# 2InfinityN6eyond/AbsoluteTrack

Hardware: AMD Instinct MI355X
Metric: hand-frames/sec (higher is better)
Workload: dtype f32 (backbone products as two fp16 pieces per operand, fp32 accumulation); 1 GPU; 4 fisheye cameras x 2 hands per frame, 2 views per hand, 96x96 crops, known-skeleton path, full hot path (resample+backbone+head+FK) + all-gather of records; frames_per_gpu=1024, src_image=480x636 u8 x 4 cameras, parallelism=frame-shard x1, world=1, backend=none (single process), outputs_finite=True

## Files before the change

### absolutetrack_amd/_native.py

```python
import contextlib
import ctypes
import os
from typing import Dict, Optional, Tuple

import numpy as np
import torch

from . import arch

_HERE = os.path.dirname(os.path.abspath(__file__))
LIB_PATH = os.path.join(_HERE, "libumetrack_hip.so")

EXPORTS = (
    "ut_weight_blob_floats", "ut_create", "ut_destroy", "ut_last_error", "ut_reserve",
    "ut_set_backbone_chunk", "ut_warp_crops", "ut_backbone", "ut_fuse_temporal_regress",
    "ut_reset_memory", "ut_get_memory", "ut_fk", "ut_gen_crop_cameras", "ut_gen_crop_matrices",
    "ut_resample_homography", "ut_keypoint_metrics", "ut_profile_begin", "ut_profile_end", "ut_profile_end_by_kind",
    "ut_set_index_checks", "ut_poll_status", "ut_warp_backbone", "ut_set_latency_mode", "ut_set_conv_arithmetic",
    "ut_set_backbone_lanes", "ut_status_snapshot", "ut_warp_map", "ut_set_block_fusion", "ut_set_resident_weights",
    "ut_canonical_backbone_weights", "ut_set_split_scale", "ut_calibrate_split", "ut_get_split_calibration",
    "ut_gen_crop_cameras_from_window_points", "ut_get_split_adaptations",
    "ut_mesh_create", "ut_mesh_destroy", "ut_mesh_counts", "ut_skin_mesh",
)

UT_MODE_KNOWN, UT_MODE_UNKNOWN = 0, 1
UT_REMAP_CV2_FIXED, UT_REMAP_FLOAT = 0, 1
UT_CHECK_SYNC, UT_CHECK_DEFERRED = 0, 1
SPLIT_SCALE_MODES = {"calibrated": 0, "dynamic": 1, "adaptive": 2}

_lib = None


class NativeLibraryError(RuntimeError):
    pass


def load_library() -> ctypes.CDLL:
    global _lib
    if _lib is not None:
        return _lib
    if not os.path.exists(LIB_PATH):
        raise NativeLibraryError(
            f"{LIB_PATH} not found: build it with `python -c 'import __graft_entry__ as g; g.build()'` "
            "(hipcc --offload-arch=gfx950).  There is no CPU fallback for the hot path.")
    lib = ctypes.CDLL(LIB_PATH)
    vp, i32, f32p = ctypes.c_void_p, ctypes.c_int, ctypes.c_void_p
    lib.ut_weight_blob_floats.restype = ctypes.c_size_t
    lib.ut_weight_blob_floats.argtypes = []
    lib.ut_create.restype = i32
    lib.ut_create.argtypes = [i32, vp, ctypes.c_size_t, ctypes.POINTER(vp)]
    lib.ut_destroy.restype = i32
    lib.ut_destroy.argtypes = [vp]
# ... 23 lines not shown
    lib.ut_mesh_destroy.restype = i32
    lib.ut_mesh_destroy.argtypes = [vp]
    lib.ut_mesh_counts.restype = i32
    lib.ut_mesh_counts.argtypes = [vp, ctypes.POINTER(i32), ctypes.POINTER(i32)]
    lib.ut_skin_mesh.restype = i32
    lib.ut_skin_mesh.argtypes = [vp, vp, f32p, i32, f32p, i32, f32p, i32, vp, ctypes.c_float, i32, f32p, f32p, vp]
    lib.ut_gen_crop_cameras.restype = i32
    lib.ut_gen_crop_cameras.argtypes = [vp, vp, vp, f32p, f32p, i32, f32p, f32p, vp, vp, i32, i32, i32, i32, i32, i32,
                                        i32, ctypes.c_double, vp, f32p, f32p, vp, vp, vp, f32p, vp]
    lib.ut_gen_crop_cameras_from_window_points.restype = i32
    lib.ut_gen_crop_cameras_from_window_points.argtypes = [vp, vp, i32, vp, vp, vp, i32, i32, i32, ctypes.c_double, vp,
                                                           f32p, f32p, vp, vp, vp, vp]
    lib.ut_gen_crop_matrices.restype = i32
    lib.ut_gen_crop_matrices.argtypes = [vp, f32p, f32p, f32p, vp, i32, i32, i32, i32, ctypes.c_double, f32p, f32p, f32p,
                                         vp, vp]
    lib.ut_resample_homography.restype = i32
    lib.ut_resample_homography.argtypes = [vp, vp, i32, i32, i32, i32, f32p, i32, i32, f32p, vp]
    lib.ut_keypoint_metrics.restype = i32
    lib.ut_keypoint_metrics.argtypes = [vp, f32p, f32p, vp, i32, i32, vp, vp, vp, vp, vp]
    lib.ut_profile_begin.restype = i32
    lib.ut_profile_begin.argtypes = [vp, vp]
    lib.ut_profile_end_by_kind.restype = i32
    lib.ut_profile_end_by_kind.argtypes = [vp, vp, ctypes.POINTER(ctypes.c_double), ctypes.POINTER(ctypes.c_int64),
                                           ctypes.POINTER(ctypes.c_double)]
    lib.ut_profile_end.restype = i32
    lib.ut_profile_end.argtypes = [vp, vp, ctypes.POINTER(ctypes.c_double), ctypes.POINTER(ctypes.c_int64),
                                   ctypes.POINTER(ctypes.c_double)]
    lib.ut_set_index_checks.restype = i32
    lib.ut_set_index_checks.argtypes = [vp, i32]
    lib.ut_set_backbone_lanes.restype = i32
    lib.ut_set_backbone_lanes.argtypes = [vp, i32]
    lib.ut_set_block_fusion.restype = i32
    lib.ut_set_block_fusion.argtypes = [vp, i32]
    lib.ut_set_resident_weights.restype = i32
    lib.ut_set_resident_weights.argtypes = [vp, i32]
    lib.ut_warp_map.restype = i32
    lib.ut_warp_map.argtypes = [vp, vp, vp, i32, i32, vp, vp]
    lib.ut_status_snapshot.restype = i32
    lib.ut_status_snapshot.argtypes = [vp, vp, vp]
    lib.ut_set_latency_mode.restype = i32
    lib.ut_set_latency_mode.argtypes = [vp, i32]
    lib.ut_set_conv_arithmetic.restype = i32
    lib.ut_set_conv_arithmetic.argtypes = [vp, i32]
    lib.ut_poll_status.restype = i32
    lib.ut_poll_status.argtypes = [vp, vp]
    lib.ut_set_split_scale.restype = i32
    lib.ut_set_split_scale.argtypes = [vp, i32]
    lib.ut_calibrate_split.restype = i32
    lib.ut_calibrate_split.argtypes = [vp, vp, i32, vp]
    lib.ut_get_split_calibration.restype = i32
    lib.ut_get_split_calibration.argtypes = [vp, vp]
    lib.ut_get_split_adaptations.restype = i32
    lib.ut_get_split_adaptations.argtypes = [vp, ctypes.POINTER(ctypes.c_uint32), i32, vp]
    lib.ut_canonical_backbone_weights.restype = i32
    lib.ut_canonical_backbone_weights.argtypes = [vp, ctypes.c_size_t, vp, ctypes.c_size_t, ctypes.POINTER(ctypes.c_size_t)]
    _lib = lib
    return lib


def state_dict_to_blob(state_dict) -> np.ndarray:
    spec = arch.state_dict_spec()
    missing = [k for k, _s, _kind in spec if k not in state_dict]
    extra = [k for k in state_dict if k not in {k for k, _s, _kind in spec}]
    if missing or extra:
        raise RuntimeError(f"Error(s) in loading state_dict: missing keys {missing[:4]}..., "
                           f"unexpected keys {extra[:4]}..." if missing or extra else "")
# ... 400 lines not shown
        self.deferred_checks = bool(deferred)

    @contextlib.contextmanager
    def modes(self, deferred_checks: Optional[bool] = None, latency: Optional[bool] = None,
              split_scale: Optional[str] = None):
        prev = (self.deferred_checks, self.latency_mode, self.split_scale)
        try:
            if deferred_checks is not None and deferred_checks != prev[0]:
                self.set_index_checks(deferred_checks)
            if latency is not None and latency != prev[1]:
                self.set_latency_mode(latency)
            if split_scale is not None and split_scale != prev[2]:
                self.set_split_scale(split_scale)
            yield self
        finally:
            if self._h:
                if self.deferred_checks != prev[0]:
                    self.set_index_checks(prev[0])
                if self.latency_mode != prev[1]:
                    self.set_latency_mode(prev[1])
                if self.split_scale != prev[2]:
                    self.set_split_scale(prev[2])

    def status_snapshot(self, out: torch.Tensor):
        out = _need(out, torch.int32, self.device, "out")
        self._check(self.lib.ut_status_snapshot(self._h, _ptr(out), _stream(self.device)), "ut_status_snapshot")

    def set_backbone_lanes(self, lanes: int):
        self._check(self.lib.ut_set_backbone_lanes(self._h, int(lanes)), "ut_set_backbone_lanes")

    def set_block_fusion(self, on: bool):
        self._check(self.lib.ut_set_block_fusion(self._h, int(bool(on))), "ut_set_block_fusion")

    def set_resident_weights(self, kind=1):
        self._check(self.lib.ut_set_resident_weights(self._h, int(kind)), "ut_set_resident_weights")

    def set_latency_mode(self, on: bool):
        self._check(self.lib.ut_set_latency_mode(self._h, int(bool(on))), "ut_set_latency_mode")
        self.latency_mode = bool(on)

    def set_conv_arithmetic(self, mode: str):
        self._check(self.lib.ut_set_conv_arithmetic(self._h, {"fp32": 0, "split_f16": 1, "split_f16_always": 2}[mode]), "ut_set_conv_arithmetic")

    def set_split_scale(self, mode: str):
        self._check(self.lib.ut_set_split_scale(self._h, SPLIT_SCALE_MODES[mode]), "ut_set_split_scale")
        self.split_scale = mode

    def split_adaptations(self, reset: bool = False) -> int:
        n = ctypes.c_uint32(0)
        self._check(self.lib.ut_get_split_adaptations(self._h, ctypes.byref(n), int(bool(reset)), _stream(self.device)),
                    "ut_get_split_adaptations")
        return int(n.value)

    def calibrate_split(self, crops: Optional[torch.Tensor] = None):
        if crops is None:
            self._check(self.lib.ut_calibrate_split(self._h, None, 0, _stream(self.device)), "ut_calibrate_split")
            return
        crops = _need(crops, torch.float32, self.device, "crops")
        if crops.ndim != 3 or tuple(crops.shape[1:]) != (arch.CROP, arch.CROP) or crops.shape[0] == 0:
            raise ValueError(f"crops must be [n >= 1,{arch.CROP},{arch.CROP}], got {tuple(crops.shape)}")
        self._check(self.lib.ut_calibrate_split(self._h, _ptr(crops), crops.shape[0], _stream(self.device)), "ut_calibrate_split")

    def split_calibration(self) -> np.ndarray:
        out = np.zeros(33, np.float32)
        self._check(self.lib.ut_get_split_calibration(self._h, out.ctypes.data_as(ctypes.c_void_p)), "ut_get_split_calibration")
        return out
# ... 140 lines not shown
```

### absolutetrack_amd/build.py

```python
import concurrent.futures
import os
import subprocess
import sys

HERE = os.path.dirname(os.path.abspath(__file__))
CSRC = os.path.join(HERE, "csrc")
OBJ = os.path.join(HERE, "_build")
OUT = os.path.join(HERE, "libumetrack_hip.so")
SOURCES = ["ut_api.hip", "conv_igemm.hip", "conv_patch.hip", "conv_block32.hip", "conv_split.hip", "conv_w4.hip", "conv_c64k.hip",
           "conv_c32s2.hip", "stem.hip", "head.hip", "fk.hip", "mesh.hip", "warp.hip", "cropgen.hip", "homography.hip", "metrics.hip"]
HEADERS = ["ut_kernels.h", "ut_math.h", "ut_fk.h", os.path.join("..", "..", "include", "umetrack_hip.h")]
FLAGS = ["--offload-arch=gfx950", "-O3", "-std=c++17", "-fPIC", "-Wall", "-Wno-unused-function"]


def _mtime(path: str) -> float:
    return os.path.getmtime(path) if os.path.exists(path) else 0.0


def _stale() -> bool:
    t = _mtime(OUT)
    return t == 0.0 or any(_mtime(os.path.join(CSRC, f)) > t for f in SOURCES + HEADERS)


def build(force: bool = False, verbose: bool = True) -> str:
    if not force and not _stale():
        return OUT
    hipcc = os.environ.get("HIPCC", "/opt/rocm/bin/hipcc")
    extra = os.environ.get("UT_EXTRA_HIPCC_FLAGS", "").split()
    os.makedirs(OBJ, exist_ok=True)
    stamp = os.path.join(OBJ, "flags.txt")
    flags_now = " ".join([hipcc] + FLAGS + extra)
    if not os.path.exists(stamp) or open(stamp).read() != flags_now:
        force = True
    newest_header = max(_mtime(os.path.join(CSRC, f)) for f in HEADERS)
    jobs = []
    for f in SOURCES:
        src, obj = os.path.join(CSRC, f), os.path.join(OBJ, f + ".o")
        if force or _mtime(obj) < max(_mtime(src), newest_header):
            jobs.append([hipcc] + FLAGS + extra + ["-c", src, "-o", obj])

    def run(cmd):
        if verbose:
            print(" ".join(cmd), flush=True)
# ... 13 lines not shown
```

### absolutetrack_amd/csrc/head.hip

```cpp
#include "ut_kernels.h"
#include "ut_math.h"

namespace ut {

constexpr int PIX = 36, FC = 72, MEMC = 18, TC = 92;

__global__ __launch_bounds__(256) void validate_desc_kernel(HeadArgs a) {
  const int s = blockIdx.x * 256 + threadIdx.x;
  if (s >= a.n_samples) return;
  int bits = 0;
  const long long r0 = a.sample_range[2 * s], r1 = a.sample_range[2 * s + 1];
  const long long nv = r1 - r0;
  if (r0 < 0 || r1 > a.n_crops || nv < 1 || nv > 2) bits |= UT_BAD_SAMPLE_RANGE;
  else if (nv == 1) bits |= UT_SINGLE_VIEW;
  const long long slot = a.memory_idx[s];
  if (slot < 0 || slot >= a.n_slots) bits |= UT_BAD_MEMORY_IDX;
  else if (atomicAdd(a.slot_seen + slot, 1) != 0) bits |= UT_DUP_MEMORY_IDX;
  const long long hand = a.hand_idx[s];
  if (hand != 0 && hand != 1) bits |= UT_BAD_HAND_IDX;
  if (bits & UT_STATUS_ERRORS) atomicOr(a.status, bits & UT_STATUS_ERRORS);
  if (bits & ~UT_STATUS_ERRORS) atomicOr(a.status + 1, bits & ~UT_STATUS_ERRORS);
}
#define UT_RETURN_IF_INVALID(a)                                                              \
  if ((((volatile const int*)(a).status)[0] & UT_STATUS_ERRORS) ||                           \
      (((volatile const int*)(a).status)[1] & (a).call_error_mask)) return

__global__ __launch_bounds__(256) void ftl_in_kernel(HeadArgs a, HeadBuffers b) {
  UT_RETURN_IF_INVALID(a);
  const int s = blockIdx.x;
  const int r0 = (int)a.sample_range[2 * s], r1 = (int)a.sample_range[2 * s + 1];
  const int nv = r1 - r0;
  __shared__ float xf[2][12];
  if (threadIdx.x < nv) {
    const int v = threadIdx.x;
    const double sv = (double)(a.intrinsics[(size_t)(r0 + v) * 9] / 200.0f);
    double out[16];
    if (nv == 1) {
      for (int i = 0; i < 16; ++i) out[i] = (i % 5 == 0) ? 1.0 : 0.0;
      out[10] = sv;
    } else {
      const double s0 = (double)(a.intrinsics[(size_t)r0 * 9] / 200.0f);
      double x0[16], xv[16], xvi[16], t[16];
      load4(a.extrinsics + (size_t)r0 * 16, x0);
      load4(a.extrinsics + (size_t)(r0 + v) * 16, xv);
      inv4(xv, xvi);
      for (int i = 0; i < 4; ++i) xvi[4 * i + 2] *= sv;
      mul4(x0, xvi, t);
      for (int j = 0; j < 4; ++j) t[8 + j] /= s0;
      for (int i = 0; i < 16; ++i) out[i] = t[i];
    }
    for (int i = 0; i < 3; ++i)
      for (int j = 0; j < 4; ++j) xf[v][4 * i + j] = (float)out[4 * i + j];
  }
  __syncthreads();
  for (int it = threadIdx.x; it < 2 * 24 * PIX; it += 256) {
    const int v = it / (24 * PIX);
    const int rem = it - v * 24 * PIX;
    const int c = rem / PIX, p = rem - c * PIX;
// ... 253 lines not shown
```

### absolutetrack_amd/csrc/ut_api.hip

```cpp
#include "../../include/umetrack_hip.h"

#include <math.h>
#include <stdio.h>
#include <stdlib.h>
#include <string.h>

#include <cmath>
#include <initializer_list>
#include <mutex>
#include <string>
#include <utility>
#include <vector>

#include "ut_kernels.h"

namespace {

thread_local std::string g_create_error;

struct ConvW {
  float* w = nullptr;
  void* w_split = nullptr;
  float split_unscale = 0.f;
  float wsum_rows = 0.f;
// ... 3 lines not shown
  int taps = 1, ksize = 1, stride = 1, pad = 0, k_total = 0, k_pad = 0, cslice = 0;
  double flops_per_pixel = 0;
};

struct Block {
  ConvW conv1, conv2, ds;
  bool has_ds = false;
};

struct Regressor {
  Block blocks[2];
  Block blocks_split[2];
  float* w_out = nullptr;
  float* b_out = nullptr;
  int c = 0, d = 0;
};

struct ProfEvent { hipEvent_t a, b; double flops;   int kind = 0;
};

}

constexpr int kDefaultChunk = 4096;
constexpr int kMaxChunk = 7281;

struct ut_context {
  int device = 0;
  int num_cu = 256;
  std::string err;
  std::vector<void*> allocs;
  float* stem_w = nullptr; float* stem_b = nullptr;
  Block bb[12];
  ConvW proj, fus0, fus1, fus2, tmp[3];
  float *skel_w = nullptr, *skel_b = nullptr, *skel_scale = nullptr, *skel_shift = nullptr;
  Regressor reg_k, reg_u;
  int chunk = kDefaultChunk;
  size_t ws_crops = 0;
  float *bufX = nullptr, *bufH = nullptr, *bufY = nullptr, *bufD = nullptr;
  size_t crops_ws_floats = 0;
  float* crops_ws = nullptr;
  size_t wsb_crops = 0;
  float *bufL2 = nullptr, *bufP = nullptr, *bufQ = nullptr, *bufBH = nullptr, *bufBD = nullptr;
  size_t ws_samples = 0;
  ut::HeadBuffers hb{};
  size_t ws_skel = 0;
  int slots_cap = 0, slots_used = 0;
  float *mem = nullptr, *prev_ext = nullptr;
  unsigned* counters = nullptr;
  int counter_next = 0;
  unsigned* calib = nullptr;
  unsigned* adapt_count = nullptr;
  int scale_mode = UT_SPLIT_SCALE_CALIBRATED;
  bool calibrated = false;
  bool head_calibrated = false;
  bool calibrating = false;
  unsigned word_gen = 0;
  bool block_fusion = true;
  int resident_weights = 1;
  bool call_split = false;
  int* status = nullptr;
  int* status_host = nullptr;
  int* slot_seen = nullptr;
  int check_mode = UT_CHECK_SYNC;
  int lanes = 1;
  hipStream_t lane_stream[2] = {nullptr, nullptr};
  hipEvent_t ev_fork = nullptr, ev_join[2] = {nullptr, nullptr};
// ... 666 lines not shown

int ut_create(int device, const float* blob, size_t n_floats, ut_handle* out) {
  if (!blob || !out) return fail(nullptr, UT_E_INVALID, "ut_create: null argument");
  if (n_floats != UT_WEIGHT_BLOB_FLOATS) return fail(nullptr, UT_E_WEIGHTS, "ut_create: weight blob has the wrong length");
  DeviceScope scope(device);
  if (scope.err != hipSuccess) return fail(nullptr, UT_E_HIP, "hipSetDevice", scope.err);
  ut_handle h = new ut_context();
  h->device = device;
  {
    int cus = 0;
    if (hipDeviceGetAttribute(&cus, hipDeviceAttributeMultiprocessorCount, device) == hipSuccess && cus > 0) h->num_cu = cus;
  }
  Cursor c{blob, n_floats};
  int rc = UT_OK;
  do {
    { float* cnt = nullptr; if ((rc = dev_alloc(h, &cnt, 2 * kMaxCounters + 64))) break; h->counters = (unsigned*)cnt;
      h->calib = h->counters + 2 * kMaxCounters;
      h->adapt_count = h->calib + 63;
      hipError_t e1 = hipMemset(h->calib, 0, 64 * sizeof(unsigned));
      if (e1 != hipSuccess) { rc = fail(h, UT_E_HIP, "calibration words", e1); break; } }
    { float* st = nullptr; if ((rc = dev_alloc(h, &st, 2))) break; h->status = (int*)st;
      hipError_t e2 = hipMemset(h->status, 0, 2 * sizeof(int));
      if (e2 == hipSuccess) e2 = hipHostMalloc((void**)&h->status_host, 2 * sizeof(int), hipHostMallocDefault);
      if (e2 != hipSuccess) { rc = fail(h, UT_E_HIP, "status words", e2); break; } }
    FoldedBackbone fbb;
    if (!fold_backbone(c, fbb)) { rc = fail(h, UT_E_WEIGHTS, "weight blob too short"); break; }
    const Folded& stem = fbb.stem;
    const Folded& proj = fbb.proj;
    const FoldedBlock* fb = fbb.fb;
    if ((rc = upload(h, stem.w, &h->stem_w)) || (rc = upload(h, stem.b, &h->stem_b))) break;
    for (int b = 0; b < 12 && !rc; ++b) rc = pack_block(h, h->bb[b], fb[b]);
    if (rc) break;
    if ((rc = pack_conv(h, h->proj, proj, 1, 1, 72))) break;
    { const float* w0 = c.take(108 * 144); const float* b0 = c.take(108); BN bn0 = take_bn(c, 108);
      const float* w1 = c.take(72 * 108); const float* b1 = c.take(72); BN bn1 = take_bn(c, 72);
      const float* w2 = c.take(72 * 72); const float* b2 = c.take(72);
      if (!c.ok) { rc = fail(h, UT_E_WEIGHTS, "weight blob too short"); break; }
      if ((rc = pack_conv(h, h->fus0, w0, b0, &bn0, 144, 108, 1, 1, 108)) ||
          (rc = pack_conv(h, h->fus1, w1, b1, &bn1, 108, 72, 1, 1, 72)) ||
          (rc = pack_conv(h, h->fus2, w2, b2, nullptr, 72, 72, 1, 1, 72))) break; }
    for (int i = 0; i < 3 && !rc; ++i) {
      const float* tw = c.take(90 * 90); const float* tb = c.take(90);
      if (!c.ok) { rc = fail(h, UT_E_WEIGHTS, "weight blob too short"); break; }
      rc = pack_conv(h, h->tmp[i], tw, tb, nullptr, 90, 90, 1, 1, 92);
    }
    if (rc) break;
    { const float* lw = c.take(144 * 132); const float* lb = c.take(144); BN bn = take_bn(c, 4);
      if (!c.ok) { rc = fail(h, UT_E_WEIGHTS, "weight blob too short"); break; }
      std::vector<float> sc(4), sh(4);
      for (int k = 0; k < 4; ++k) {
        double s = (double)bn.g[k] / sqrt((double)bn.v[k] + 1e-5);
        sc[k] = (float)s; sh[k] = (float)((double)bn.b[k] - (double)bn.m[k] * s);
      }
      if ((rc = upload(h, std::vector<float>(lw, lw + 144 * 132), &h->skel_w)) ||
          (rc = upload(h, std::vector<float>(lb, lb + 144), &h->skel_b)) ||
          (rc = upload(h, sc, &h->skel_scale)) || (rc = upload(h, sh, &h->skel_shift))) break; }
    if ((rc = take_regressor(h, c, h->reg_k, 76, 62))) break;
    if ((rc = take_regressor(h, c, h->reg_u, 72, 63))) break;
    if (!c.ok || c.left != 0) { rc = fail(h, UT_E_WEIGHTS, "weight blob length does not match the architecture"); break; }
  } while (0);
  if (rc) {
    g_create_error = h->err;
    ut_destroy(h);
    return rc;
  }
  *out = h;
  return UT_OK;
}

int ut_destroy(ut_handle h) {
  if (!h) return UT_OK;
  DeviceScope scope(h->device);
  (void)hipDeviceSynchronize();
  for (void* p : h->allocs) (void)hipFree(p);
  if (h->status_host) (void)hipHostFree(h->status_host);
  for (int i = 0; i < 2; ++i) {
    if (h->lane_stream[i]) (void)hipStreamDestroy(h->lane_stream[i]);
    if (h->ev_join[i]) (void)hipEventDestroy(h->ev_join[i]);
  }
// ... 281 lines not shown
int ut_backbone(ut_handle h, const float* crops, int n_crops, float* feat, void* stream) {
  if (!h) return UT_E_INVALID;
  if (n_crops == 0) return UT_OK;
  if (!crops || !feat || n_crops < 0) return fail(h, UT_E_INVALID, "ut_backbone: bad argument");
  ON_DEVICE_OF(h);
  return run_backbone(h, crops, nullptr, n_crops, feat, (hipStream_t)stream);
}

int ut_warp_backbone(ut_handle h, const uint8_t* src, int n_src_images, int src_h, int src_w, const double* cam_params,
                     const double* crop_params, const int32_t* src_index, int n_crops, int remap_mode, float* feat,
                     void* stream) {
  if (!h) return UT_E_INVALID;
  if (n_crops == 0) return UT_OK;
  if (!src || !cam_params || !crop_params || !src_index || !feat || n_crops < 0 || src_h <= 0 || src_w <= 0 ||
      n_src_images <= 0 || (remap_mode != UT_REMAP_CV2_FIXED && remap_mode != UT_REMAP_FLOAT))
    return fail(h, UT_E_INVALID, "ut_warp_backbone: bad argument");
  ON_DEVICE_OF(h);
  hipStream_t s = (hipStream_t)stream;
  const bool u8 = remap_mode == UT_REMAP_CV2_FIXED;
  int rc = regrow(h, &h->crops_ws_floats, (size_t)n_crops * 96 * 96 / (u8 ? sizeof(float) : 1), {{&h->crops_ws, 1}});
  if (rc) return rc;
  HIPCHK(h, ut::launch_warp(src, n_src_images, src_h, src_w, cam_params, crop_params, src_index, n_crops, remap_mode,
                            u8 ? nullptr : h->crops_ws, u8 ? (uint8_t*)h->crops_ws : nullptr, h->status, s));
  if (h->check_mode == UT_CHECK_SYNC && (rc = check_status(h, h->status, h->status_host, s, "ut_warp_backbone"))) return rc;
  return run_backbone(h, u8 ? nullptr : h->crops_ws, u8 ? (const uint8_t*)h->crops_ws : nullptr, n_crops, feat, s);
}

static int run_head(ut_handle h, const ut::HeadArgs& a, const float* skel, int n_skel, int mode, float* out_pose, float* out_raw,
                    hipStream_t s) {
  int rc;
  const ut::HeadBuffers& b = h->hb;
  const int S = a.n_samples;
  h->call_split = false;
  HIPCHK(h, ut::launch_ftl_in(a, b, s));
  if ((rc = run_conv(h, h->fus0, b.cat144, nullptr, b.f108, S, 6, 6, true, false, s))) return rc;
  if ((rc = run_conv(h, h->fus1, b.f108, nullptr, b.f72a, S, 6, 6, true, false, s))) return rc;
  if ((rc = run_conv(h, h->fus2, b.f72a, nullptr, b.f72b, S, 6, 6, false, false, s))) return rc;
  HIPCHK(h, ut::launch_ftl_out_temporal_in(a, b, s));
  if ((rc = run_conv(h, h->tmp[0], b.t92a, nullptr, b.t92b, S, 6, 6, true, false, s))) return rc;
  if ((rc = run_conv(h, h->tmp[1], b.t92b, nullptr, b.t92a, S, 6, 6, true, false, s))) return rc;
  if ((rc = run_conv(h, h->tmp[2], b.t92a, nullptr, b.t92b, S, 6, 6, false, false, s))) return rc;
  const Regressor& reg = mode == UT_MODE_KNOWN_SKELETON ? h->reg_k : h->reg_u;
  if (mode == UT_MODE_KNOWN_SKELETON)
    HIPCHK(h, ut::launch_skeleton(skel, h->skel_w, h->skel_b, h->skel_scale, h->skel_shift, b.skel, n_skel, s));
  const bool head_split = !h->latency_mode && (h->calibrating || h->scale_mode == UT_SPLIT_SCALE_DYNAMIC || h->head_calibrated) &&
                          (h->conv_arith == UT_CONV_SPLIT_F16_ALWAYS || (h->conv_arith == UT_CONV_SPLIT_F16 && S >= 4 * h->num_cu));
  const int stride = head_split ? kRegSplitCh : reg.c;
  const int tid0 = mode == UT_MODE_KNOWN_SKELETON ? 25 : 29;
  unsigned* in_word = nullptr;
  if (head_split) {
    int word = 0;
    if (h->counter_next + 16 > kMaxCounters && (rc = begin_call(h, s))) return rc;
    if ((rc = next_launch_word(h, s, &word))) return rc;
    in_word = h->counters + kMaxCounters + word;
  }
  HIPCHK(h, ut::launch_temporal_out(a, b.t92b, b.skel, n_skel, b.regin, reg.c, stride, in_word, s));
  h->call_split = head_split;
  const Block* blocks = head_split ? reg.blocks_split : reg.blocks;
  unsigned* mid_word = nullptr;
  rc = run_block(h, blocks[0], b.regin, b.rega, nullptr, b.regb, S, 6, 6, s, in_word, &mid_word, head_split ? tid0 : -1, head_split ? tid0 + 1 : -1);
  if (!rc) rc = run_block(h, blocks[1], b.regb, b.rega, nullptr, b.regin, S, 6, 6, s, mid_word, nullptr, head_split ? tid0 + 2 : -1, head_split ? tid0 + 3 : -1);
  h->call_split = false;
  if (rc) return rc;
  HIPCHK(h, ut::launch_pool_decode(a, b.regin, reg.c, stride, reg.w_out, reg.b_out, reg.d, out_pose, out_raw, b.rega, s));
  return UT_OK;
}

int ut_fuse_temporal_regress(ut_handle h, const float* feat, const float* intrinsics, const float* extrinsics,
                             const int64_t* sample_range, const int64_t* memory_idx, const uint8_t* use_memory,
                             const int64_t* hand_idx, int n_crops, int n_samples, int n_slots, int all_multiview,
                             const float* skel, int n_skel, int mode, float* out_pose, float* out_raw, void* stream) {
  if (!h) return UT_E_INVALID;
  if (n_samples == 0) return UT_OK;
  if (!feat || !intrinsics || !extrinsics || !sample_range || !memory_idx || !use_memory || !hand_idx || !out_pose ||
      n_samples < 0 || n_crops < n_samples || n_crops > 2 * n_samples || n_slots <= 0)
    return fail(h, UT_E_INVALID, "ut_fuse_temporal_regress: bad argument");
  if (mode == UT_MODE_KNOWN_SKELETON) {
    if (!skel || (n_skel != 1 && n_skel != n_samples))
      return fail(h, UT_E_INVALID, "ut_fuse_temporal_regress: skeleton must have 1 or n_samples entries");
  } else if (mode == UT_MODE_UNKNOWN_SKELETON) {
    if (!all_multiview)
      return fail(h, UT_E_UNSUPPORTED, "Unsupported: found single-view samples when calibration scale");
    n_skel = 0;
  } else {
    return fail(h, UT_E_INVALID, "ut_fuse_temporal_regress: unknown mode");
  }
  ON_DEVICE_OF(h);
  hipStream_t s = (hipStream_t)stream;
  int rc;
// ... 267 lines not shown
                        double* err, double* acc, double* gt_acc, uint8_t* valid_acc, void* stream) {
  if (n_hands == 0 || n_frames == 0) return UT_OK;
  if (!gt || !tracked || !valid || !err || n_hands < 0 || n_frames < 0 ||
      (n_frames >= 3 && (!acc || !gt_acc || !valid_acc)))
    return fail(h, UT_E_INVALID, "ut_keypoint_metrics: bad argument");
  ON_DEVICE_IF(h);
  HIPCHK(h, ut::launch_keypoint_metrics(gt, tracked, valid, n_hands, n_frames, err, acc, gt_acc, valid_acc,
                                        (hipStream_t)stream));
  return UT_OK;
}

int ut_set_backbone_lanes(ut_handle h, int lanes) {
  if (!h || (lanes != 1 && lanes != 2)) return fail(h, UT_E_INVALID, "ut_set_backbone_lanes: 1 or 2");
  h->lanes = lanes;
  return UT_OK;
}

int ut_set_conv_arithmetic(ut_handle h, int mode) {
  if (!h || (mode != UT_CONV_FP32 && mode != UT_CONV_SPLIT_F16 && mode != UT_CONV_SPLIT_F16_ALWAYS)) return fail(h, UT_E_INVALID, "ut_set_conv_arithmetic: bad argument");
  h->conv_arith = mode;
  if (mode != UT_CONV_FP32 && h->scale_mode != UT_SPLIT_SCALE_DYNAMIC && !h->calibrated) {
    ON_DEVICE_OF(h);
    return calibrate_builtin(h);
  }
  return UT_OK;
}

int ut_set_block_fusion(ut_handle h, int on) {
  if (!h) return UT_E_INVALID;
  h->block_fusion = on != 0;
  return UT_OK;
}

int ut_set_resident_weights(ut_handle h, int on) {
  if (!h) return UT_E_INVALID;
  if (on < 0 || on > 6) return fail(h, UT_E_INVALID, "ut_set_resident_weights: bad argument");
  h->resident_weights = on;
  return UT_OK;
}

int ut_set_latency_mode(ut_handle h, int on) {
  if (!h) return UT_E_INVALID;
  ON_DEVICE_OF(h);
  if (on && !h->splitk_ws) {
    const size_t n = 1u << 20;
    int rc;
    if ((rc = dev_alloc(h, &h->splitk_ws, n)) || (rc = dev_alloc(h, &h->zero_bias, 256))) return rc;
    HIPCHK(h, hipMemset(h->zero_bias, 0, 256 * sizeof(float)));
    h->splitk_floats = n;
  }
  h->latency_mode = on != 0;
  return UT_OK;
}

int ut_set_index_checks(ut_handle h, int mode) {
  if (!h || (mode != UT_CHECK_SYNC && mode != UT_CHECK_DEFERRED)) return fail(h, UT_E_INVALID, "ut_set_index_checks: bad argument");
  h->check_mode = mode;
  return UT_OK;
}

int ut_poll_status(ut_handle h, void* stream) {
  if (!h) return UT_E_INVALID;
  ON_DEVICE_OF(h);
  return check_status(h, h->status, h->status_host, (hipStream_t)stream, "reported late (deferred checks)");
}

// ... 37 lines not shown
```

### absolutetrack_amd/csrc/ut_kernels.h

```cpp
#pragma once
#include <hip/hip_runtime.h>
#include <stdint.h>

namespace ut {

struct ConvLaunch {
  const float* in;
  const float* w;
  const void* w_split;
  float split_unscale;
  int* status;
  const unsigned* in_max;
  const unsigned* in_obs;
  int split_adaptive;
  unsigned* adapt_count;
  unsigned* out_max;
  const float* bias;
  const float* res;
  float* out;
  int n_img, H, W, cin, Ho, Wo;
  int cout_store;
  int cout_pad;
  int k_total;
  int cslice;
// ... 130 lines not shown
  ok = e != 255;
  scale = __uint_as_float((unsigned)(127 + k) << 23);
  unscale = __uint_as_float((unsigned)(127 - k) << 23);
  if (in_obs && !adapted && (eo == 255 || eo + k > 142)) ok = false;
  return bits;
}

__device__ __forceinline__ void split_scale_report(bool ok, bool adapted, int* status, unsigned* adapt_count) {
  if (threadIdx.x == 0 && blockIdx.x == 0) {
    if (!ok && status) atomicOr(status, UT_SPLIT_RANGE);
    if (adapted && adapt_count) atomicAdd(adapt_count, 1u);
  }
}
#endif

struct HeadArgs {
  const float* feat;
  const float* intrinsics;
  const float* extrinsics;
  const int64_t* sample_range;
  const int64_t* memory_idx;
  const uint8_t* use_memory;
  const int64_t* hand_idx;
  int n_samples;
  int n_crops;
  int n_slots;
  float* mem;
  float* prev_ext;
  int* status;
  int call_error_mask;
  int* slot_seen;
};

hipError_t launch_validate_desc(const HeadArgs& a, hipStream_t s);

hipError_t launch_ftl_in(const HeadArgs& a, const HeadBuffers& b, hipStream_t s);
hipError_t launch_ftl_out_temporal_in(const HeadArgs& a, const HeadBuffers& b, hipStream_t s);
hipError_t launch_temporal_out(const HeadArgs& a, const float* t_out , const float* skel,
                               int n_skel, float* regin, int reg_c, int reg_stride, unsigned* out_max, hipStream_t s);
hipError_t launch_skeleton(const float* skel_in , const float* w ,
                           const float* bias , const float* bn_scale ,
                           const float* bn_shift , float* out , int n_skel,
                           hipStream_t s);
hipError_t launch_pool_decode(const HeadArgs& a, const float* reg_feat , int reg_c, int reg_stride,
                              const float* w , const float* bias , int d,
                              float* out_pose, float* out_raw, float* raw_ws , hipStream_t s);

hipError_t launch_fk(const float* hand_model, int n_models, const float* ja, int ja_stride,
                     const float* xf, int xf_stride, const int64_t* mirror, float t_scale, int n,
                     float* out, hipStream_t s);

constexpr int MESH_MAX_VERTICES = 5056;
hipError_t launch_skin_mesh(const float* hand_model, int n_models, const float* ja, int ja_stride, const float* xf,
                            int xf_stride, const int64_t* mirror, float t_scale, int n, const void* verts,
                            const uint32_t* csr_off, const uint32_t* csr_ent, int nv, float* out_v, float* out_n,
                            hipStream_t s);

struct CropGenArgs {
  const double* cam_params;
  const double* camera_angles;
  const float* hand_model;
  const float* joint_limits;
  const float* joint_angles;
  const float* wrist_xf;
  const int32_t* frame_idx;
  const int64_t* hand_idx;
  int n, n_models, n_cams, max_views, min_vis, src_w, src_h, crop_size;
  double focal_multiplier;
  double* crop_params;
  float* intrinsics;
  float* extrinsics;
  int32_t* cam_index;
  int32_t* n_views;
  int32_t* status;
  float* landmarks;
};
hipError_t launch_cropgen(const CropGenArgs& g, hipStream_t s);

struct CropGenWindowArgs {
// ... 45 lines not shown
```

### include/umetrack_hip.h

```cpp
#ifndef UMETRACK_HIP_H
#define UMETRACK_HIP_H

#include <stddef.h>
#include <stdint.h>

#ifdef __cplusplus
extern "C" {
#endif

typedef struct ut_context* ut_handle;

enum {
  UT_OK = 0,
  UT_E_INVALID = -1,
  UT_E_HIP = -2,
  UT_E_WEIGHTS = -3,
  UT_E_UNSUPPORTED = -4
};

enum { UT_MODE_KNOWN_SKELETON = 0, UT_MODE_UNKNOWN_SKELETON = 1 };
enum { UT_CHECK_SYNC = 0, UT_CHECK_DEFERRED = 1 };
enum { UT_REMAP_CV2_FIXED = 0, UT_REMAP_FLOAT = 1 };

#define UT_CROP 96
#define UT_FEAT_CH 72
#define UT_FEAT_PIX 36
#define UT_POSE_REC 60
#define UT_CAM_PARAMS 32
#define UT_CROP_PARAMS 24
#define UT_HAND_MODEL_FLOATS 321
#define UT_WEIGHT_BLOB_FLOATS 4259410

size_t ut_weight_blob_floats(void);

int ut_create(int device, const float* weights_blob, size_t n_floats, ut_handle* out);

int ut_canonical_backbone_weights(const float* weights_blob, size_t n_floats, float* out, size_t out_floats, size_t* n_out);
int ut_destroy(ut_handle h);
const char* ut_last_error(ut_handle h);

int ut_set_index_checks(ut_handle h, int mode);
int ut_poll_status(ut_handle h, void* stream);
int ut_status_snapshot(ut_handle h, int32_t* dst, void* stream);

int ut_set_backbone_lanes(ut_handle h, int lanes);

enum { UT_CONV_FP32 = 0, UT_CONV_SPLIT_F16 = 1, UT_CONV_SPLIT_F16_ALWAYS = 2 };
int ut_set_conv_arithmetic(ut_handle h, int mode);

enum { UT_SPLIT_SCALE_CALIBRATED = 0, UT_SPLIT_SCALE_DYNAMIC = 1, UT_SPLIT_SCALE_CALIBRATED_ADAPTIVE = 2 };
int ut_set_split_scale(ut_handle h, int mode);
int ut_get_split_adaptations(ut_handle h, uint32_t* out, int reset, void* stream);
int ut_calibrate_split(ut_handle h, const float* crops, int n_crops, void* stream);
int ut_get_split_calibration(ut_handle h, float* out33);

int ut_set_block_fusion(ut_handle h, int on);

int ut_set_resident_weights(ut_handle h, int on);

int ut_set_latency_mode(ut_handle h, int on);

int ut_reserve(ut_handle h, int max_crops, int max_samples, int max_slots);

int ut_set_backbone_chunk(ut_handle h, int crops_per_pass);

int ut_warp_crops(ut_handle h, const uint8_t* src, int n_src_images, int src_h, int src_w,
                  const double* cam_params, const double* crop_params, const int32_t* src_index,
                  int n_crops, int remap_mode, float* out, void* stream);

int ut_warp_map(const double* cam_params, const double* crop_params, const int32_t* src_index, int n_src_images,
                int n_crops, float* out_map, void* stream);

int ut_backbone(ut_handle h, const float* crops, int n_crops, float* feat, void* stream);

int ut_warp_backbone(ut_handle h, const uint8_t* src, int n_src_images, int src_h, int src_w,
                     const double* cam_params, const double* crop_params, const int32_t* src_index,
                     int n_crops, int remap_mode, float* feat, void* stream);

int ut_fuse_temporal_regress(ut_handle h, const float* feat, const float* intrinsics,
                             const float* extrinsics, const int64_t* sample_range,
                             const int64_t* memory_idx, const uint8_t* use_memory,
                             const int64_t* hand_idx, int n_crops, int n_samples, int n_slots,
                             int all_multiview, const float* skel, int n_skel, int mode,
                             float* out_pose, float* out_raw, void* stream);

int ut_reset_memory(ut_handle h);
int ut_get_memory(ut_handle h, float* mem, float* prev_ext, int max_slots, void* stream);

int ut_fk(ut_handle h, const float* hand_model, int n_models, const float* joint_angles,
// ... 53 lines not shown
```

Baseline: 163,200 hand-frames/s.

## Fuse temporal head 1x1 conv chain into single LDS-resident MFMA kernel

Adds a head_chain kernel that, for groups of three samples, computes the view-fusion transform, runs the six 1x1 head convolutions (fusion and temporal layers) with fp32 MFMA on activations kept in shared memory, applies the memory update, and writes regressor input directly. It replaces the ftl_in, six separate conv launches and temporal_out with one launch, removing intermediate global round-trips and launch overhead. It is on by default outside latency mode. In exchange it uses about 75KB of LDS per block, which limits occupancy, and runs the head in plain fp32 instead of the split-f16 conv path.

After: 163,600 hand-frames/s (median of 6 runs). About the same (+0.2%).

```diff
diff --git a/absolutetrack_amd/_native.py b/absolutetrack_amd/_native.py
--- a/absolutetrack_amd/_native.py
+++ b/absolutetrack_amd/_native.py
@@ -18,6 +18,7 @@
     "ut_resample_homography", "ut_keypoint_metrics", "ut_profile_begin", "ut_profile_end", "ut_profile_end_by_kind",
     "ut_set_index_checks", "ut_poll_status", "ut_warp_backbone", "ut_set_latency_mode", "ut_set_conv_arithmetic",
     "ut_set_backbone_lanes", "ut_status_snapshot", "ut_warp_map", "ut_set_block_fusion", "ut_set_resident_weights",
+    "ut_set_head_chain",
     "ut_canonical_backbone_weights", "ut_set_split_scale", "ut_calibrate_split", "ut_get_split_calibration",
     "ut_gen_crop_cameras_from_window_points", "ut_get_split_adaptations",
     "ut_mesh_create", "ut_mesh_destroy", "ut_mesh_counts", "ut_skin_mesh",
@@ -107,6 +108,8 @@
     lib.ut_set_backbone_lanes.argtypes = [vp, i32]
     lib.ut_set_block_fusion.restype = i32
     lib.ut_set_block_fusion.argtypes = [vp, i32]
+    lib.ut_set_head_chain.restype = i32
+    lib.ut_set_head_chain.argtypes = [vp, i32]
     lib.ut_set_resident_weights.restype = i32
     lib.ut_set_resident_weights.argtypes = [vp, i32]
     lib.ut_warp_map.restype = i32
@@ -573,6 +576,9 @@
     def set_block_fusion(self, on: bool):
         self._check(self.lib.ut_set_block_fusion(self._h, int(bool(on))), "ut_set_block_fusion")
 
+    def set_head_chain(self, on: bool):
+        self._check(self.lib.ut_set_head_chain(self._h, int(bool(on))), "ut_set_head_chain")
+
     def set_resident_weights(self, kind=1):
         self._check(self.lib.ut_set_resident_weights(self._h, int(kind)), "ut_set_resident_weights")
 
diff --git a/absolutetrack_amd/build.py b/absolutetrack_amd/build.py
--- a/absolutetrack_amd/build.py
+++ b/absolutetrack_amd/build.py
@@ -8,7 +8,7 @@
 OBJ = os.path.join(HERE, "_build")
 OUT = os.path.join(HERE, "libumetrack_hip.so")
 SOURCES = ["ut_api.hip", "conv_igemm.hip", "conv_patch.hip", "conv_block32.hip", "conv_split.hip", "conv_w4.hip", "conv_c64k.hip",
-           "conv_c32s2.hip", "stem.hip", "head.hip", "fk.hip", "mesh.hip", "warp.hip", "cropgen.hip", "homography.hip", "metrics.hip"]
+           "conv_c32s2.hip", "stem.hip", "head.hip", "head_chain.hip", "fk.hip", "mesh.hip", "warp.hip", "cropgen.hip", "homography.hip", "metrics.hip"]
 HEADERS = ["ut_kernels.h", "ut_math.h", "ut_fk.h", os.path.join("..", "..", "include", "umetrack_hip.h")]
 FLAGS = ["--offload-arch=gfx950", "-O3", "-std=c++17", "-fPIC", "-Wall", "-Wno-unused-function"]
 
diff --git a/absolutetrack_amd/csrc/head.hip b/absolutetrack_amd/csrc/head.hip
--- a/absolutetrack_amd/csrc/head.hip
+++ b/absolutetrack_amd/csrc/head.hip
@@ -21,9 +21,6 @@
   if (bits & UT_STATUS_ERRORS) atomicOr(a.status, bits & UT_STATUS_ERRORS);
   if (bits & ~UT_STATUS_ERRORS) atomicOr(a.status + 1, bits & ~UT_STATUS_ERRORS);
 }
-#define UT_RETURN_IF_INVALID(a)                                                              \
-  if ((((volatile const int*)(a).status)[0] & UT_STATUS_ERRORS) ||                           \
-      (((volatile const int*)(a).status)[1] & (a).call_error_mask)) return
 
 __global__ __launch_bounds__(256) void ftl_in_kernel(HeadArgs a, HeadBuffers b) {
   UT_RETURN_IF_INVALID(a);
diff --git a/absolutetrack_amd/csrc/head_chain.hip b/absolutetrack_amd/csrc/head_chain.hip
--- /dev/null
+++ b/absolutetrack_amd/csrc/head_chain.hip
@@ -0,0 +1,262 @@
+#include <atomic>
+
+#include "ut_kernels.h"
+#include "ut_math.h"
+
+namespace ut {
+
+namespace {
+
+typedef float f32x16 __attribute__((ext_vector_type(16)));
+
+constexpr int PIX = 36, FC = 72, MEMC = 18;
+constexpr int G = HEAD_CHAIN_SAMPLES;
+constexpr int ROWS = 128;
+constexpr int LD = 148;
+constexpr int T_COLS = 96;
+static_assert(G * PIX <= ROWS, "every sample row needs an owner");
+
+template <int NC, int KG>
+__device__ __forceinline__ void conv_rows(float* act, const float* __restrict__ wl, int rb, int lane, bool relu, int coff) {
+  const int fr = lane & 31, fh = lane >> 5;
+  const float* __restrict__ bias = wl + (size_t)NC * KG * 256;
+  f32x16 acc[NC];
+#pragma unroll
+  for (int j = 0; j < NC; ++j)
+#pragma unroll
+    for (int g4 = 0; g4 < 4; ++g4) {
+      const float4 b = *reinterpret_cast<const float4*>(bias + j * 32 + 8 * g4 + 4 * fh);
+      acc[j][4 * g4 + 0] = b.x + 0.f;
+      acc[j][4 * g4 + 1] = b.y + 0.f;
+      acc[j][4 * g4 + 2] = b.z + 0.f;
+      acc[j][4 * g4 + 3] = b.w + 0.f;
+    }
+  const float* px = act + (rb * 32 + fr) * LD + 4 * fh;
+  const float4* __restrict__ wp = reinterpret_cast<const float4*>(wl) + lane;
+  float4 wn[NC], pn;
+#pragma unroll
+  for (int j = 0; j < NC; ++j) wn[j] = wp[(j * KG) * 64];
+  pn = *reinterpret_cast<const float4*>(px);
+#pragma unroll 2
+  for (int q = 0; q < KG; ++q) {
+    float4 wc[NC];
+#pragma unroll
+    for (int j = 0; j < NC; ++j) wc[j] = wn[j];
+    const float4 pc = pn;
+    if (q + 1 < KG) {
+#pragma unroll
+      for (int j = 0; j < NC; ++j) wn[j] = wp[(j * KG + q + 1) * 64];
+      pn = *reinterpret_cast<const float4*>(px + 8 * (q + 1));
+    }
+#pragma unroll
+    for (int j = 0; j < NC; ++j) acc[j] = __builtin_amdgcn_mfma_f32_32x32x2f32(wc[j].x, pc.x, acc[j], 0, 0, 0);
+#pragma unroll
+    for (int j = 0; j < NC; ++j) acc[j] = __builtin_amdgcn_mfma_f32_32x32x2f32(wc[j].y, pc.y, acc[j], 0, 0, 0);
+#pragma unroll
+    for (int j = 0; j < NC; ++j) acc[j] = __builtin_amdgcn_mfma_f32_32x32x2f32(wc[j].z, pc.z, acc[j], 0, 0, 0);
+#pragma unroll
+    for (int j = 0; j < NC; ++j) acc[j] = __builtin_amdgcn_mfma_f32_32x32x2f32(wc[j].w, pc.w, acc[j], 0, 0, 0);
+  }
+  const float floor_v = relu ? 0.f : -__builtin_huge_valf();
+  float* orow = act + (rb * 32 + fr) * LD + coff + 4 * fh;
+#pragma unroll
+  for (int j = 0; j < NC; ++j)
+#pragma unroll
+    for (int g4 = 0; g4 < 4; ++g4) {
+      float* o = orow + j * 32 + 8 * g4;
+      const float v0 = fmaxf(acc[j][4 * g4 + 0], floor_v), v1 = fmaxf(acc[j][4 * g4 + 1], floor_v);
+      const float v2 = fmaxf(acc[j][4 * g4 + 2], floor_v), v3 = fmaxf(acc[j][4 * g4 + 3], floor_v);
+      if ((coff & 3) == 0) *reinterpret_cast<float4*>(o) = make_float4(v0, v1, v2, v3);
+      else { o[0] = v0; o[1] = v1; o[2] = v2; o[3] = v3; }
+    }
+}
+
+template <int L>
+__device__ __forceinline__ void conv_layer(float* act, const float* __restrict__ blob, int rb, int lane, bool relu, int coff) {
+  conv_rows<head_chain_blocks(L), head_chain_kgroups(L)>(act, blob + head_chain_offset(L), rb, lane, relu, coff);
+}
+
+}
+
+__global__ __launch_bounds__(256, 2) void head_chain_kernel(HeadArgs a, HeadChainArgs c) {
+  UT_RETURN_IF_INVALID(a);
+  extern __shared__ __attribute__((aligned(16))) float act[];
+  __shared__ float xf[G][2][12];
+  __shared__ float rel[G][12];
+  const int tid = threadIdx.x, lane = tid & 63;
+  const int wave = __builtin_amdgcn_readfirstlane(tid >> 6);
+  const int s_first = blockIdx.x * G;
+  const int ns = a.n_samples - s_first < G ? a.n_samples - s_first : G;
+
+  if (tid < 2 * G && (tid >> 1) < ns) {
+    const int g = tid >> 1, v = tid & 1, s = s_first + g;
+    const int r0 = (int)a.sample_range[2 * s], r1 = (int)a.sample_range[2 * s + 1];
+    const int nv = r1 - r0;
+    if (v < nv) {
+      const double sv = (double)(a.intrinsics[(size_t)(r0 + v) * 9] / 200.0f);
+      double out[16];
+      if (nv == 1) {
+        for (int i = 0; i < 16; ++i) out[i] = (i % 5 == 0) ? 1.0 : 0.0;
+        out[10] = sv;
+      } else {
+        const double s0 = (double)(a.intrinsics[(size_t)r0 * 9] / 200.0f);
+        double x0[16], xv[16], xvi[16], t[16];
+        load4(a.extrinsics + (size_t)r0 * 16, x0);
+        load4(a.extrinsics + (size_t)(r0 + v) * 16, xv);
+        inv4(xv, xvi);
+        for (int i = 0; i < 4; ++i) xvi[4 * i + 2] *= sv;
+        mul4(x0, xvi, t);
+        for (int j = 0; j < 4; ++j) t[8 + j] /= s0;
+        for (int i = 0; i < 16; ++i) out[i] = t[i];
+      }
+      for (int i = 0; i < 3; ++i)
+        for (int j = 0; j < 4; ++j) xf[g][v][4 * i + j] = (float)out[4 * i + j];
+    }
+  } else if (tid >= 64 && tid < 64 + ns) {
+    const int g = tid - 64, s = s_first + g;
+    const int r0 = (int)a.sample_range[2 * s];
+    const int slot = (int)a.memory_idx[s];
+    double cur[16];
+    load4(a.extrinsics + (size_t)r0 * 16, cur);
+    if (a.use_memory[s] != 0) {
+      double prev[16], pinv[16], r[16];
+      load4(a.prev_ext + (size_t)slot * 16, prev);
+      inv4(prev, pinv);
+      mul4(cur, pinv, r);
+      for (int i = 0; i < 12; ++i) rel[g][i] = (float)r[i];
+    }
+    for (int i = 0; i < 16; ++i) a.prev_ext[(size_t)slot * 16 + i] = (float)cur[i];
+  }
+  __syncthreads();
+
+  for (int g = 0; g < ns; ++g) {
+    const int s = s_first + g;
+    const int r0 = (int)a.sample_range[2 * s], r1 = (int)a.sample_range[2 * s + 1];
+    const int nv = r1 - r0;
+    for (int it = tid; it < 2 * 24 * PIX; it += 256) {
+      const int v = it / (24 * PIX);
+      const int rem = it - v * 24 * PIX;
+      const int ch = rem / PIX, p = rem - ch * PIX;
+      float* o144 = act + (g * PIX + p) * LD + v * FC;
+      if (nv == 2) {
+        const float* f = a.feat + (size_t)(r0 + v) * FC * PIX;
+        const float x = f[ch * PIX + p], y = f[(24 + ch) * PIX + p], z = f[(48 + ch) * PIX + p];
+        const float* m = xf[g][v];
+        o144[ch] = m[0] * x + m[1] * y + m[2] * z + m[3];
+        o144[24 + ch] = m[4] * x + m[5] * y + m[6] * z + m[7];
+        o144[48 + ch] = m[8] * x + m[9] * y + m[10] * z + m[11];
+      } else {
+        o144[ch] = 0.f; o144[24 + ch] = 0.f; o144[48 + ch] = 0.f;
+        if (v == 0) {
+          const float* f = a.feat + (size_t)r0 * FC * PIX;
+          const float* m = xf[g][0];
+          const float x = f[ch * PIX + p], y = f[(24 + ch) * PIX + p], z = f[(48 + ch) * PIX + p];
+          float* o = c.fused + ((size_t)s * PIX + p) * FC;
+          o[ch] = m[0] * x + m[1] * y + m[2] * z + m[3];
+          o[24 + ch] = m[4] * x + m[5] * y + m[6] * z + m[7];
+          o[48 + ch] = m[8] * x + m[9] * y + m[10] * z + m[11];
+        }
+      }
+    }
+  }
+  __syncthreads();
+
+  conv_layer<0>(act, c.w, wave, lane, true, 0);
+  conv_layer<1>(act, c.w, wave, lane, true, 0);
+  conv_layer<2>(act, c.w, wave, lane, false, MEMC);
+  __syncthreads();
+
+  for (int g = 0; g < ns; ++g) {
+    const int s = s_first + g;
+    const int r0 = (int)a.sample_range[2 * s], r1 = (int)a.sample_range[2 * s + 1];
+    const int nv = r1 - r0;
+    const int slot = (int)a.memory_idx[s];
+    const bool use_mem = a.use_memory[s] != 0;
+    const float s0 = a.intrinsics[(size_t)r0 * 9] / 200.0f;
+    for (int it = tid; it < PIX * T_COLS; it += 256) {
+      const int p = it / T_COLS, ch = it - p * T_COLS;
+      float* row = act + (g * PIX + p) * LD;
+      float v = 0.f;
+      if (ch >= MEMC && ch < MEMC + FC) {
+        const int fc = ch - MEMC;
+        const size_t o = ((size_t)s * PIX + p) * FC + fc;
+        if (nv == 2) {
+          v = row[ch];
+          if (fc >= 48) v *= s0;
+          c.fused[o] = v;
+        } else {
+          v = c.fused[o];
+        }
+      } else if (ch < MEMC && use_mem) {
+        const float* m = a.mem + ((size_t)slot * PIX + p) * MEMC;
+        const int k = ch % 6, r = ch / 6;
+        v = rel[g][4 * r] * m[k] + rel[g][4 * r + 1] * m[6 + k] + rel[g][4 * r + 2] * m[12 + k] + rel[g][4 * r + 3];
+      }
+      row[ch] = v;
+    }
+  }
+  __syncthreads();
+
+  conv_layer<3>(act, c.w, wave, lane, true, 0);
+  conv_layer<4>(act, c.w, wave, lane, true, 0);
+  conv_layer<5>(act, c.w, wave, lane, false, 0);
+  __syncthreads();
+
+  unsigned mx = 0;
+  for (int g = 0; g < ns; ++g) {
+    const int s = s_first + g;
+    const int slot = (int)a.memory_idx[s];
+    for (int it = tid; it < PIX * MEMC; it += 256) {
+      const int p = it / MEMC, ch = it - p * MEMC;
+      a.mem[((size_t)slot * PIX + p) * MEMC + ch] = act[(g * PIX + p) * LD + ch];
+    }
+    const float* sk = c.reg_c > FC ? c.skel + (size_t)(c.n_skel == 1 ? 0 : s) * PIX * 4 : nullptr;
+    float* ro = c.regin + (size_t)s * PIX * c.reg_stride;
+    for (int it = tid; it < PIX * c.reg_stride; it += 256) {
+      const int p = it / c.reg_stride, ch = it - p * c.reg_stride;
+      float v = 0.f;
+      if (ch < FC) {
+        v = act[(g * PIX + p) * LD + MEMC + ch];
+        mx = max(mx, abs_bits(v));
+      } else if (ch < c.reg_c) {
+        v = sk[p * 4 + (ch - FC)];
+        mx = max(mx, abs_bits(v));
+      }
+      ro[it] = v;
+    }
+  }
+  if (c.out_max) publish_abs_max(c.out_max, mx);
+}
+
+hipError_t launch_head_chain(const HeadArgs& a, const HeadChainArgs& c, hipStream_t s) {
+  if (a.n_samples <= 0 || !c.w || !c.fused || !c.regin || c.reg_c < FC || c.reg_c > FC + 4 || c.reg_stride < c.reg_c ||
+      (c.reg_c > FC && (!c.skel || (c.n_skel != 1 && c.n_skel != a.n_samples))))
+    return hipErrorInvalidValue;
+  constexpr size_t lds = (size_t)ROWS * LD * sizeof(float);
+  static std::atomic<unsigned long long> attr_set{0};
+  const unsigned long long dev_bit = (c.device >= 0 && c.device < 64) ? 1ull << c.device : 0ull;
+  if (!(attr_set.load(std::memory_order_relaxed) & dev_bit) || !dev_bit) {
+    hipError_t e = hipFuncSetAttribute(reinterpret_cast<const void*>(&head_chain_kernel),
+                                       hipFuncAttributeMaxDynamicSharedMemorySize, (int)lds);
+    if (e != hipSuccess) return e;
+    attr_set.fetch_or(dev_bit, std::memory_order_relaxed);
+  }
+  hipLaunchKernelGGL(head_chain_kernel, dim3((a.n_samples + G - 1) / G), dim3(256), lds, s, a, c);
+  return hipGetLastError();
+}
+
+void head_chain_pack_layer(int l, const float* w, const float* bias, float* blob) {
+  const int cin = head_chain_cin(l), cout = head_chain_cout(l), kg = head_chain_kgroups(l), nc = head_chain_blocks(l);
+  float* wl = blob + head_chain_offset(l);
+  float* bl = wl + (size_t)nc * kg * 256;
+  for (int cb = 0; cb < nc; ++cb)
+    for (int q = 0; q < kg; ++q)
+      for (int ln = 0; ln < 64; ++ln)
+        for (int e = 0; e < 4; ++e) {
+          const int o = cb * 32 + (ln & 31), k = 8 * q + 4 * (ln >> 5) + e;
+          wl[(((size_t)cb * kg + q) * 64 + ln) * 4 + e] = (o < cout && k < cin) ? w[(size_t)o * cin + k] : 0.f;
+        }
+  for (int o = 0; o < nc * 32; ++o) bl[o] = o < cout ? bias[o] : 0.f;
+}
+
+}
diff --git a/absolutetrack_amd/csrc/ut_api.hip b/absolutetrack_amd/csrc/ut_api.hip
--- a/absolutetrack_amd/csrc/ut_api.hip
+++ b/absolutetrack_amd/csrc/ut_api.hip
@@ -59,6 +59,8 @@
   float* stem_w = nullptr; float* stem_b = nullptr;
   Block bb[12];
   ConvW proj, fus0, fus1, fus2, tmp[3];
+  float* head_chain_w = nullptr;
+  bool head_chain = true;
   float *skel_w = nullptr, *skel_b = nullptr, *skel_scale = nullptr, *skel_shift = nullptr;
   Regressor reg_k, reg_u;
   int chunk = kDefaultChunk;
@@ -791,19 +793,25 @@
     for (int b = 0; b < 12 && !rc; ++b) rc = pack_block(h, h->bb[b], fb[b]);
     if (rc) break;
     if ((rc = pack_conv(h, h->proj, proj, 1, 1, 72))) break;
+    std::vector<float> chain_blob(ut::HEAD_CHAIN_BLOB_FLOATS, 0.f);
     { const float* w0 = c.take(108 * 144); const float* b0 = c.take(108); BN bn0 = take_bn(c, 108);
       const float* w1 = c.take(72 * 108); const float* b1 = c.take(72); BN bn1 = take_bn(c, 72);
       const float* w2 = c.take(72 * 72); const float* b2 = c.take(72);
       if (!c.ok) { rc = fail(h, UT_E_WEIGHTS, "weight blob too short"); break; }
-      if ((rc = pack_conv(h, h->fus0, w0, b0, &bn0, 144, 108, 1, 1, 108)) ||
-          (rc = pack_conv(h, h->fus1, w1, b1, &bn1, 108, 72, 1, 1, 72)) ||
-          (rc = pack_conv(h, h->fus2, w2, b2, nullptr, 72, 72, 1, 1, 72))) break; }
+      const Folded f0 = fold_conv(w0, b0, &bn0, 144, 108, 1), f1 = fold_conv(w1, b1, &bn1, 108, 72, 1), f2 = fold_conv(w2, b2, nullptr, 72, 72, 1);
+      if ((rc = pack_conv(h, h->fus0, f0, 1, 1, 108)) || (rc = pack_conv(h, h->fus1, f1, 1, 1, 72)) || (rc = pack_conv(h, h->fus2, f2, 1, 1, 72))) break;
+      ut::head_chain_pack_layer(0, f0.w.data(), f0.b.data(), chain_blob.data());
+      ut::head_chain_pack_layer(1, f1.w.data(), f1.b.data(), chain_blob.data());
+      ut::head_chain_pack_layer(2, f2.w.data(), f2.b.data(), chain_blob.data()); }
     for (int i = 0; i < 3 && !rc; ++i) {
       const float* tw = c.take(90 * 90); const float* tb = c.take(90);
       if (!c.ok) { rc = fail(h, UT_E_WEIGHTS, "weight blob too short"); break; }
-      rc = pack_conv(h, h->tmp[i], tw, tb, nullptr, 90, 90, 1, 1, 92);
+      const Folded ft = fold_conv(tw, tb, nullptr, 90, 90, 1);
+      rc = pack_conv(h, h->tmp[i], ft, 1, 1, 92);
+      ut::head_chain_pack_layer(3 + i, ft.w.data(), ft.b.data(), chain_blob.data());
     }
     if (rc) break;
+    if ((rc = upload(h, chain_blob, &h->head_chain_w))) break;
     { const float* lw = c.take(144 * 132); const float* lb = c.take(144); BN bn = take_bn(c, 4);
       if (!c.ok) { rc = fail(h, UT_E_WEIGHTS, "weight blob too short"); break; }
       std::vector<float> sc(4), sh(4);
@@ -1151,6 +1159,29 @@
   const ut::HeadBuffers& b = h->hb;
   const int S = a.n_samples;
   h->call_split = false;
+  const Regressor& reg = mode == UT_MODE_KNOWN_SKELETON ? h->reg_k : h->reg_u;
+  const bool head_split = !h->latency_mode && (h->calibrating || h->scale_mode == UT_SPLIT_SCALE_DYNAMIC || h->head_calibrated) &&
+                          (h->conv_arith == UT_CONV_SPLIT_F16_ALWAYS || (h->conv_arith == UT_CONV_SPLIT_F16 && S >= 4 * h->num_cu));
+  const int stride = head_split ? kRegSplitCh : reg.c;
+  const int tid0 = mode == UT_MODE_KNOWN_SKELETON ? 25 : 29;
+  unsigned* in_word = nullptr;
+  const bool chain = h->head_chain && !h->latency_mode;
+  if (chain) {
+    if (mode == UT_MODE_KNOWN_SKELETON)
+      HIPCHK(h, ut::launch_skeleton(skel, h->skel_w, h->skel_b, h->skel_scale, h->skel_shift, b.skel, n_skel, s));
+    if (head_split) {
+      int word = 0;
+      if (h->counter_next + 16 > kMaxCounters && (rc = begin_call(h, s))) return rc;
+      if ((rc = next_launch_word(h, s, &word))) return rc;
+      in_word = h->counters + kMaxCounters + word;
+    }
+    ut::HeadChainArgs hc{};
+    hc.w = h->head_chain_w; hc.skel = b.skel; hc.n_skel = n_skel; hc.fused = b.fused; hc.regin = b.regin;
+    hc.reg_c = reg.c; hc.reg_stride = stride; hc.out_max = in_word; hc.device = h->device;
+    double flops = 0;
+    for (const ConvW* cw : {&h->fus0, &h->fus1, &h->fus2, &h->tmp[0], &h->tmp[1], &h->tmp[2]}) flops += cw->flops_per_pixel * (double)S * 36;
+    if ((rc = bracket_launch(h, s, -1, nullptr, flops, 0, "launch_head_chain", [&] { return ut::launch_head_chain(a, hc, s); }))) return rc;
+  } else {
   HIPCHK(h, ut::launch_ftl_in(a, b, s));
   if ((rc = run_conv(h, h->fus0, b.cat144, nullptr, b.f108, S, 6, 6, true, false, s))) return rc;
   if ((rc = run_conv(h, h->fus1, b.f108, nullptr, b.f72a, S, 6, 6, true, false, s))) return rc;
@@ -1159,14 +1190,8 @@
   if ((rc = run_conv(h, h->tmp[0], b.t92a, nullptr, b.t92b, S, 6, 6, true, false, s))) return rc;
   if ((rc = run_conv(h, h->tmp[1], b.t92b, nullptr, b.t92a, S, 6, 6, true, false, s))) return rc;
   if ((rc = run_conv(h, h->tmp[2], b.t92a, nullptr, b.t92b, S, 6, 6, false, false, s))) return rc;
-  const Regressor& reg = mode == UT_MODE_KNOWN_SKELETON ? h->reg_k : h->reg_u;
   if (mode == UT_MODE_KNOWN_SKELETON)
     HIPCHK(h, ut::launch_skeleton(skel, h->skel_w, h->skel_b, h->skel_scale, h->skel_shift, b.skel, n_skel, s));
-  const bool head_split = !h->latency_mode && (h->calibrating || h->scale_mode == UT_SPLIT_SCALE_DYNAMIC || h->head_calibrated) &&
-                          (h->conv_arith == UT_CONV_SPLIT_F16_ALWAYS || (h->conv_arith == UT_CONV_SPLIT_F16 && S >= 4 * h->num_cu));
-  const int stride = head_split ? kRegSplitCh : reg.c;
-  const int tid0 = mode == UT_MODE_KNOWN_SKELETON ? 25 : 29;
-  unsigned* in_word = nullptr;
   if (head_split) {
     int word = 0;
     if (h->counter_next + 16 > kMaxCounters && (rc = begin_call(h, s))) return rc;
@@ -1174,6 +1199,7 @@
     in_word = h->counters + kMaxCounters + word;
   }
   HIPCHK(h, ut::launch_temporal_out(a, b.t92b, b.skel, n_skel, b.regin, reg.c, stride, in_word, s));
+  }
   h->call_split = head_split;
   const Block* blocks = head_split ? reg.blocks_split : reg.blocks;
   unsigned* mid_word = nullptr;
@@ -1507,6 +1533,12 @@
   return UT_OK;
 }
 
+int ut_set_head_chain(ut_handle h, int on) {
+  if (!h) return UT_E_INVALID;
+  h->head_chain = on != 0;
+  return UT_OK;
+}
+
 int ut_set_resident_weights(ut_handle h, int on) {
   if (!h) return UT_E_INVALID;
   if (on < 0 || on > 6) return fail(h, UT_E_INVALID, "ut_set_resident_weights: bad argument");
diff --git a/absolutetrack_amd/csrc/ut_kernels.h b/absolutetrack_amd/csrc/ut_kernels.h
--- a/absolutetrack_amd/csrc/ut_kernels.h
+++ b/absolutetrack_amd/csrc/ut_kernels.h
@@ -186,6 +186,10 @@
   int* slot_seen;
 };
 
+#define UT_RETURN_IF_INVALID(a)                                                              \
+  if ((((volatile const int*)(a).status)[0] & UT_STATUS_ERRORS) ||                           \
+      (((volatile const int*)(a).status)[1] & (a).call_error_mask)) return
+
 hipError_t launch_validate_desc(const HeadArgs& a, hipStream_t s);
 
 hipError_t launch_ftl_in(const HeadArgs& a, const HeadBuffers& b, hipStream_t s);
@@ -199,6 +203,28 @@
 hipError_t launch_pool_decode(const HeadArgs& a, const float* reg_feat , int reg_c, int reg_stride,
                               const float* w , const float* bias , int d,
                               float* out_pose, float* out_raw, float* raw_ws , hipStream_t s);
+
+constexpr int HEAD_CHAIN_SAMPLES = 3;
+constexpr int HEAD_CHAIN_LAYERS = 6;
+constexpr int head_chain_cin(int l) { return l == 0 ? 144 : l == 1 ? 108 : l == 2 ? 72 : 90; }
+constexpr int head_chain_cout(int l) { return l == 0 ? 108 : l < 3 ? 72 : 90; }
+constexpr int head_chain_kgroups(int l) { return l == 0 ? 18 : l == 1 ? 14 : l == 2 ? 9 : 12; }
+constexpr int head_chain_blocks(int l) { return l == 0 ? 4 : 3; }
+constexpr size_t head_chain_layer_floats(int l) { return (size_t)head_chain_blocks(l) * (head_chain_kgroups(l) * 256 + 32); }
+constexpr size_t head_chain_offset(int l) { return l == 0 ? 0 : head_chain_offset(l - 1) + head_chain_layer_floats(l - 1); }
+constexpr size_t HEAD_CHAIN_BLOB_FLOATS = head_chain_offset(HEAD_CHAIN_LAYERS);
+void head_chain_pack_layer(int l, const float* w, const float* bias, float* blob);
+struct HeadChainArgs {
+  const float* w;
+  const float* skel;
+  int n_skel;
+  float* fused;
+  float* regin;
+  int reg_c, reg_stride;
+  unsigned* out_max;
+  int device;
+};
+hipError_t launch_head_chain(const HeadArgs& a, const HeadChainArgs& c, hipStream_t s);
 
 hipError_t launch_fk(const float* hand_model, int n_models, const float* ja, int ja_stride,
                      const float* xf, int xf_stride, const int64_t* mirror, float t_scale, int n,
diff --git a/include/umetrack_hip.h b/include/umetrack_hip.h
--- a/include/umetrack_hip.h
+++ b/include/umetrack_hip.h
@@ -55,6 +55,8 @@
 int ut_get_split_calibration(ut_handle h, float* out33);
 
 int ut_set_block_fusion(ut_handle h, int on);
+
+int ut_set_head_chain(ut_handle h, int on);
 
 int ut_set_resident_weights(ut_handle h, int on);
 
```
